# lukedan/libfluid

Measured on AMD Instinct MI355X. Metric: particle_steps_per_sec, higher is better.
Workload: dtype f32

## Files before the change

libfluid_amd/csrc/particles.hip:

```cpp
#include <math.h>

#include <algorithm>
#include <utility>

#include "common.h"
#include "pcg.h"

namespace {

__device__ inline bool solid_or_outside(const GridDims &g, const uint8_t *solid, int x, int y, int z) {
	if (!in_grid(g, x, y, z)) return true;
	return solid[blocked_index(g, x, y, z)] != 0;
}

__device__ inline void collide(const GridDims &g, const uint8_t *solid, double from[3], double to[3], double skin) {
	for (int bounce = 0; bounce < 3; ++bounce) {
		bool hit = false;
		double diff[3], inv[3], t[3];
		int cur[3], last[3], adv[3];
#pragma unroll
		for (int d = 0; d < 3; ++d) {
			cur[d] = (int)floor(from[d]);
			last[d] = (int)floor(to[d]);
			diff[d] = to[d] - from[d];
// ... 177 lines not shown
k_advect_collide(size_t n, ParticleSoA p, GridDims g, const uint8_t *solid, MoveParams mp, const uint8_t *coerce_map,
                 const float *src_vel, const uint8_t *tile_clear) {
	const size_t i = (size_t)blockIdx.x * blockDim.x + threadIdx.x;
	if (i < n) advect_one<COERCE>(i, p, g, solid, mp, coerce_map, src_vel, tile_clear);
}

#define AC_CHUNKS 8
template <bool COERCE>
__global__ void __launch_bounds__(256)
k_advect_collide_count(size_t n, ParticleSoA p, GridDims g, const uint8_t *solid, MoveParams mp, const uint8_t *coerce_map,
                       const float *src_vel, const uint8_t *tile_clear, uint32_t *tile_count, uint32_t *rank) {
	const int lane = threadIdx.x & 63;
	const size_t wave = ((size_t)blockIdx.x * blockDim.x + threadIdx.x) >> 6;
	const size_t i0 = wave * (64 * AC_CHUNKS) + lane;
	uint32_t tile[AC_CHUNKS], my_rank[AC_CHUNKS];
#pragma unroll
	for (int c = 0; c < AC_CHUNKS; ++c) {
		const size_t i = i0 + 64 * c;
		const uint32_t k = i < n ? advect_one<COERCE>(i, p, g, solid, mp, coerce_map, src_vel, tile_clear) : 0xFFFFFFFFu;
		tile[c] = k != 0xFFFFFFFFu ? k >> 9 : 0xFFFFFFFFu;
	}
	lfa_wave_tile_ranks(tile, tile_count, my_rank);
#pragma unroll
	for (int c = 0; c < AC_CHUNKS; ++c) {
		const size_t i = i0 + 64 * c;
		if (tile[c] != 0xFFFFFFFFu) rank[i] = my_rank[c];
	}
}

__device__ inline float hash_unit(uint32_t a, uint32_t b, uint32_t k) {
	uint32_t x = a * 0x9E3779B1u ^ (b + 0x7F4A7C15u) * 0x85EBCA77u ^ k * 0xC2B2AE3Du;
	x ^= x >> 15; x *= 0x2C1B3C6Du; x ^= x >> 12; x *= 0x297A2D39u; x ^= x >> 15;
	return (float)(x >> 8) * (2.0f / 16777216.0f) - 1.0f;
}

#define FT 11
#define FTX (2 * FT)
#define FT3 (FTX * FT * FT)
#define FT_STRIDE (FT3 + 1)
#define FT_INV 1.375f
#define FTX_INV 2.75f
#define FT_PL ((FT + CORR_PARTS - 1) / CORR_PARTS)
#define FB 13
#define FBX (FTX + 4)
#define FBZ (FT_PL + 2)
#define FB_N (FBX * FB * FBZ)
#define FB_ROWS (FB * FBZ)
#define FINE_CAP 5632
#define FINE_CAP_BIG 12288
#define FIDX_THREADS 512
#define FIDX_CNT (((FT3 + 1 + FIDX_THREADS - 1) / FIDX_THREADS) * FIDX_THREADS)
#define FIDX_STAGE 4608

__device__ inline int fine_coord(int l, float t) {
	const int f = (int)(((float)l + t) * FT_INV);
	return f < FT - 1 ? f : FT - 1;
}
__device__ inline int fine_coord_x(int l, float t) {
	const int f = (int)(((float)l + t) * FTX_INV);
	return f < FTX - 1 ? f : FTX - 1;
}
__device__ inline float4 fine_record(int lx, int ly, int lz, float t0, float t1, float t2, uint32_t index) {
	const uint32_t b0 = (__float_as_uint(t0) & 0x3FFFFFFFu) | ((uint32_t)(lx & 3) << 30);
	const uint32_t b1 = (__float_as_uint(t1) & 0x3FFFFFFFu) | ((uint32_t)(lx >> 2) << 31) | ((uint32_t)(ly & 1) << 30);
	const uint32_t b2 = (__float_as_uint(t2) & 0x3FFFFFFFu) | ((uint32_t)(lz & 1) << 31);
	return make_float4(__uint_as_float(b0), __uint_as_float(b1), __uint_as_float(b2), __uint_as_float(index));
}
__device__ inline void fine_decode_at(const float4 &r, int y0, int z0, float t[3], int l[3]) {
	const uint32_t b0 = __float_as_uint(r.x), b1 = __float_as_uint(r.y), b2 = __float_as_uint(r.z);
	t[0] = __uint_as_float(b0 & 0x3FFFFFFFu); t[1] = __uint_as_float(b1 & 0x3FFFFFFFu); t[2] = __uint_as_float(b2 & 0x3FFFFFFFu);
	l[0] = (int)(b0 >> 30) | ((int)(b1 >> 31) << 2);
	l[1] = y0 + ((y0 ^ (int)(b1 >> 30)) & 1);
	l[2] = z0 + ((z0 ^ (int)(b2 >> 31)) & 1);
}
__device__ inline void fine_decode(const float4 &r, int fy, int fz, float t[3], int l[3]) {
	fine_decode_at(r, (8 * fy) / FT, (8 * fz) / FT, t, l);
}

__global__ void __launch_bounds__(FIDX_THREADS)
k_build_fine_index(const int *ptiles, int n_ptiles, const uint32_t *key, const float *t0, const float *t1, const float *t2,
                   const uint32_t *tile_start, const uint32_t *tile_count, uint32_t *fine_start, float4 *spos, uint32_t *key_copy) {
	__shared__ uint32_t cnt[FIDX_CNT / 2];
	__shared__ uint32_t wsum[FIDX_THREADS / 64];
	__shared__ float4 stage[FIDX_STAGE];
	static_assert(FIDX_CNT % (2 * FIDX_THREADS) == 0 && FIDX_STAGE % FIDX_THREADS == 0 && FIDX_STAGE < 65536 && FIDX_CNT <= 4 * FIDX_STAGE,
	              "index kernel sizing");
	constexpr int PER = FIDX_CNT / FIDX_THREADS;
	uint32_t *cnt_big = (uint32_t *)stage;
	auto fine_of = [&](uint32_t i, int l[3], float t[3]) -> int {
		const uint32_t k = key[i];
		l[0] = (int)(k & 7); l[1] = (int)((k >> 3) & 7); l[2] = (int)((k >> 6) & 7);
		t[0] = t0[i]; t[1] = t1[i]; t[2] = t2[i];
		return fine_coord_x(l[0], t[0]) + FTX * (fine_coord(l[1], t[1]) + FT * fine_coord(l[2], t[2]));
	};
	constexpr int RPT = FIDX_STAGE / FIDX_THREADS;
	for (int slot = blockIdx.x; slot < n_ptiles; slot += gridDim.x) {
		const int tile = ptiles[slot];
		const uint32_t b = tile_start[tile], e = b + tile_count[tile];
		const bool staged = e - b <= FIDX_STAGE;
		if (staged) {
#pragma unroll
			for (int k = 0; k < PER / 2; ++k) cnt[threadIdx.x + FIDX_THREADS * k] = 0;
		} else {
#pragma unroll
			for (int k = 0; k < PER; ++k) cnt_big[threadIdx.x + FIDX_THREADS * k] = 0;
		}
		__syncthreads();
		uint32_t rf[RPT];
		float r0[RPT], r1[RPT], r2[RPT];
		if (staged) {
#pragma unroll
			for (int r = 0; r < RPT; ++r) {
				const uint32_t i = b + threadIdx.x + FIDX_THREADS * r;
				rf[r] = 0xFFFFFFFFu;
				if (i < e) {
					int l[3];
					float t[3];
					const int f = fine_of(i, l, t);
					rf[r] = ((uint32_t)f << 9) | (uint32_t)(l[0] | (l[1] << 3) | (l[2] << 6));
					r0[r] = t[0]; r1[r] = t[1]; r2[r] = t[2];
					atomicAdd(&cnt[f >> 1], 1u << (16 * (f & 1)));
				}
			}
		} else {
			for (uint32_t i = b + threadIdx.x; i < e; i += FIDX_THREADS) {
				int l[3];
				float t[3];
				atomicAdd(&cnt_big[fine_of(i, l, t)], 1u);
			}
		}
		__syncthreads();
		uint32_t c[PER], incl = 0;
#pragma unroll
		for (int k = 0; k < PER; ++k) {
			c[k] = staged ? (cnt[(PER / 2) * threadIdx.x + k / 2] >> (16 * (k & 1))) & 0xFFFFu : cnt_big[PER * threadIdx.x + k];
			incl += c[k];
		}
		const uint32_t sum = incl;
		const int lane = threadIdx.x & 63, wid = threadIdx.x >> 6;
#pragma unroll
		for (int o = 1; o < 64; o <<= 1) {
			uint32_t t = __shfl_up(incl, o, 64);
			if (lane >= o) incl += t;
		}
		if (lane == 63) wsum[wid] = incl;
		__syncthreads();
		uint32_t ex = incl - sum;
		for (int w = 0; w < wid; ++w) ex += wsum[w];
		__syncthreads();
#pragma unroll
		for (int k = 0; k < PER; ++k) {
			const int f = PER * threadIdx.x + k;
			if (!staged) cnt_big[f] = ex;
			else if (k & 1) cnt[f >> 1] = (ex - c[k - (k & 1)]) | (ex << 16);
			if (!staged && f <= FT3) fine_start[(size_t)tile * FT_STRIDE + f] = b + ex;
			ex += c[k];
		}
		__syncthreads();
		if (staged) {
#pragma unroll
			for (int r = 0; r < RPT; ++r)
				if (rf[r] != 0xFFFFFFFFu) {
					const uint32_t f = rf[r] >> 9;
					const uint32_t at = (atomicAdd(&cnt[f >> 1], 1u << (16 * (f & 1))) >> (16 * (f & 1))) & 0xFFFFu;
					stage[at] = fine_record((int)(rf[r] & 7), (int)((rf[r] >> 3) & 7), (int)((rf[r] >> 6) & 7), r0[r], r1[r], r2[r],
					                        b + threadIdx.x + FIDX_THREADS * r);
				}
			if (key_copy) {
#pragma unroll
				for (int r = 0; r < RPT; ++r)
					if (rf[r] != 0xFFFFFFFFu) key_copy[b + threadIdx.x + FIDX_THREADS * r] = ((uint32_t)tile << 9) | (rf[r] & 511u);
			}
			__syncthreads();
			for (int f = threadIdx.x; f <= FT3; f += FIDX_THREADS)
				fine_start[(size_t)tile * FT_STRIDE + f] = b + (f ? (cnt[(f - 1) >> 1] >> (16 * ((f - 1) & 1))) & 0xFFFFu : 0u);
			for (uint32_t k = threadIdx.x; k < e - b; k += FIDX_THREADS) spos[b + k] = stage[k];
		} else {
			for (uint32_t i = b + threadIdx.x; i < e; i += FIDX_THREADS) {
				int l[3];
				float t[3];
				const uint32_t at = atomicAdd(&cnt_big[fine_of(i, l, t)], 1u);
				spos[b + at] = fine_record(l[0], l[1], l[2], t[0], t[1], t[2], i);
				if (key_copy) key_copy[i] = key[i];
			}
		}
		__syncthreads();
	}
}

__device__ inline int fine_source(const GridDims &g, const uint32_t *tile_count, int tx, int ty, int tz, int gx, int gy, int gz, int &fx,
                                  int &fy, int &fz) {
	const int dx = gx < 0 ? -1 : (gx >= FTX ? 1 : 0), dy = gy < 0 ? -1 : (gy >= FT ? 1 : 0), dz = gz < 0 ? -1 : (gz >= FT ? 1 : 0);
	fx = gx - FTX * dx; fy = gy - FT * dy; fz = gz - FT * dz;
	const int x = tx + dx, y = ty + dy, z = tz + dz;
	if ((unsigned)x >= (unsigned)g.ntx || (unsigned)y >= (unsigned)g.nty || (unsigned)z >= (unsigned)g.ntz) return -1;
	const int tile = x + g.ntx * (y + g.nty * z);
	return tile_count[tile] ? tile : -1;
}

__device__ inline void correct_collide_record(size_t rk, const ParticleSoA &p, uint32_t *out_key, float *out_tx, float *out_ty, float *out_tz,
                                              const GridDims &g, const uint8_t *solid, const uint32_t *tile_count, const uint32_t *fine_start,
                                              const float4 *spos, const MoveParams &mp, const uint32_t *only_flagged, const int *tile_pslot,
                                              int p_off, const uint32_t *key_before) {
	const float4 me = spos[rk];
	const size_t i = __float_as_uint(me.w);
	const uint32_t key_i = key_before ? key_before[i] : p.key[i];
	if (key_i == 0xFFFFFFFFu) return;
	const int tile = (int)(key_i >> 9);
	const int l[3] = {(int)(key_i & 7), (int)((key_i >> 3) & 7), (int)((key_i >> 6) & 7)};
	const float t[3] = {__uint_as_float(__float_as_uint(me.x) & 0x3FFFFFFFu), __uint_as_float(__float_as_uint(me.y) & 0x3FFFFFFFu),
	                    __uint_as_float(__float_as_uint(me.z) & 0x3FFFFFFFu)};
	const int f[3] = {fine_coord_x(l[0], t[0]), fine_coord(l[1], t[1]), fine_coord(l[2], t[2])};
	if (only_flagged) {
		const int work = CORR_PARTS * (tile_pslot[tile] - p_off) + f[2] / FT_PL;
		if (!((only_flagged[1 + (work >> 5)] >> (work & 31)) & 1u)) return;
	}
	int tx, ty, tz;
	tile_coords(g, tile, tx, ty, tz);
	const int nn[3] = {g.nx, g.ny, g.nz};
	const float inv_re2 = (float)mp.inv_re2;
	double spring[3] = {0.0, 0.0, 0.0};
	for (int dz = -1; dz <= 1; ++dz)
		for (int dy = -1; dy <= 1; ++dy)
			for (int dx = -2; dx <= 2; ++dx) {
				int sf[3];
				const int src = fine_source(g, tile_count, tx, ty, tz, f[0] + dx, f[1] + dy, f[2] + dz, sf[0], sf[1], sf[2]);
				if (src < 0) continue;
				const uint32_t *fs = fine_start + (size_t)src * FT_STRIDE + (sf[0] + FTX * (sf[1] + FT * sf[2]));
				const uint32_t kb = fs[0], ke = fs[1];
				int stx, sty, stz;
				tile_coords(g, src, stx, sty, stz);
				for (uint32_t k = kb; k < ke; ++k) {
					const float4 rec = spos[k];
					if (__float_as_uint(rec.w) == (uint32_t)i) continue;
					float nt[3];
					int nl[3];
					fine_decode(rec, sf[1], sf[2], nt, nl);
					const float ddx = ((float)(8 * (tx - stx) + l[0] - nl[0]) + t[0]) - nt[0];
					const float ddy = ((float)(8 * (ty - sty) + l[1] - nl[1]) + t[1]) - nt[1];
					const float ddz = ((float)(8 * (tz - stz) + l[2] - nl[2]) + t[2]) - nt[2];
					const float d2 = ddx * ddx + ddy * ddy + ddz * ddz;
					if (d2 < 1e-12f) {
						const uint32_t j = __float_as_uint(rec.w);
						spring[0] += hash_unit((uint32_t)i, j, 0); spring[1] += hash_unit((uint32_t)i, j, 1);
						spring[2] += hash_unit((uint32_t)i, j, 2);
					} else {
						const float kl = 1.0f - d2 * inv_re2;
						if (kl > 0.0f) {
							const float fr = kl * kl * kl * rsqrtf(d2);
							spring[0] += (double)(fr * ddx); spring[1] += (double)(fr * ddy); spring[2] += (double)(fr * ddz);
						}
					}
				}
			}
	const int c[3] = {8 * tx + l[0], 8 * ty + l[1], 8 * tz + l[2]};
	double from[3], to[3];
#pragma unroll
	for (int d = 0; d < 3; ++d) {
		from[d] = (double)c[d] + (double)t[d];
		double x = from[d] + spring[d] * mp.corr;
		to[d] = x < 0.0 ? 0.0 : ((double)nn[d] < x ? (double)nn[d] : x);
	}
	if (mp.collide) collide(g, solid, from, to, mp.skin);
	int nc[3];
	float ntt[3];
#pragma unroll
	for (int d = 0; d < 3; ++d) split_position(to[d], nn[d], nc[d], ntt[d]);
	out_key[i] = blocked_index(g, nc[0], nc[1], nc[2]);
	out_tx[i] = ntt[0]; out_ty[i] = ntt[1]; out_tz[i] = ntt[2];
}

__global__ void __launch_bounds__(256)
k_correct_collide(size_t n, ParticleSoA p, uint32_t *out_key, float *out_tx, float *out_ty, float *out_tz, GridDims g,
                   const uint8_t *solid, const uint32_t *tile_count, const uint32_t *fine_start, const float4 *spos, MoveParams mp,
                   const uint32_t *only_flagged, const int *tile_pslot, int p_off, const uint32_t *key_before) {
	if (only_flagged && only_flagged[0] == 0) return;
	for (size_t rk = (size_t)blockIdx.x * blockDim.x + threadIdx.x; rk < n; rk += (size_t)gridDim.x * blockDim.x)
		correct_collide_record(rk, p, out_key, out_tx, out_ty, out_tz, g, solid, tile_count, fine_start, spos, mp, only_flagged, tile_pslot,
		                       p_off, key_before);
}

#ifdef CORR_PROFILE
__device__ unsigned long long g_corr_prof[8];
#define CORR_STAMP(k)                                                                   \
	do {                                                                                \
		if (!ONLY && threadIdx.x == 0) {                                                \
			const unsigned long long now_ = wall_clock64();                             \
			atomicAdd(&g_corr_prof[k], now_ - stamp_);                                  \
			stamp_ = now_;                                                              \
		}                                                                               \
	} while (0)
#else
#define CORR_STAMP(k) do { } while (0)
#endif
template <int CAP, bool ONLY>
__global__ void __launch_bounds__(ONLY ? CORR_THREADS_BIG : CORR_THREADS, 4)
k_correct_fine(const int *ptiles, int n_ptiles, uint32_t *out_key, float *out_tx, float *out_ty, float *out_tz, GridDims g,
                const uint8_t *solid, const uint32_t *tile_count, const uint32_t *fine_start, const float4 *spos, MoveParams mp,
                uint32_t *overflow_tiles, const uint8_t *tile_clear, const uint32_t *only) {
	constexpr int T = ONLY ? CORR_THREADS_BIG : CORR_THREADS;
	constexpr int CNT0 = ((FB_N + 1 + 2 * T - 1) / (2 * T)) * (2 * T);
	constexpr int CNT = ONLY && CNT0 < 4096 ? 4096 : CNT0;
	__shared__ float px[CAP], py[CAP], pz[CAP];
	__shared__ uint32_t fcnt2[CNT / 2];
	uint16_t *fcnt = (uint16_t *)fcnt2;
	__shared__ uint16_t foff[FB_N + 1];
	__shared__ __attribute__((aligned(16))) uint32_t rowd[FB_ROWS * 4];
	__shared__ uint32_t rowe[FB_ROWS];
	constexpr int ROW_NOT_OWN = -32768;
	__shared__ uint32_t ownoff[FT * FT_PL + 1];
	__shared__ int srct[27];
	__shared__ uint32_t wsum[T / 64];
	uint16_t *own = fcnt;
	static_assert(CNT > FB_N && CNT % (2 * T) == 0 && FBX % 2 == 0 && CAP < 32768 && CNT < 32768, "fcnt sizing");
	constexpr int PER = CNT / T;
	const int nn[3] = {g.nx, g.ny, g.nz};
	const int lane = threadIdx.x & 63, wid = threadIdx.x >> 6;
	if (ONLY && only[0] == 0) return;
	constexpr int SLICES = ONLY ? CORR_BIG_SLICES : 1;
	for (int item = blockIdx.x; item < SLICES * CORR_PARTS * n_ptiles; item += gridDim.x) {
		const int work = item / SLICES, slice = item % SLICES;
		if (ONLY && !((only[1 + (work >> 5)] >> (work & 31)) & 1u)) continue;
		const int tile = ptiles[work / CORR_PARTS], part = work % CORR_PARTS;
		int tx, ty, tz;
		tile_coords(g, tile, tx, ty, tz);
		const int own_lo = part * FT_PL, own_n = (own_lo + FT_PL <= FT ? FT_PL : FT - own_lo);
		const int gz0 = own_lo - 1;
		const int nzb = own_n + 2;
		const int nrows = FB * nzb, nown_rows = FT * (nzb - 2);
		const bool open_water = (tile_clear[tile] & 1) != 0;
		const bool lean = open_water && mp.collide && tx >= 1 && ty >= 1 && tz >= 1 && 8 * tx + 16 <= g.nx && 8 * ty + 16 <= g.ny &&
		                  8 * tz + 16 <= g.nz;
		__syncthreads();
#ifdef CORR_PROFILE
		unsigned long long stamp_ = wall_clock64();
		if (!ONLY && threadIdx.x == 0) atomicAdd(&g_corr_prof[7], 1ull);
#endif
		uint32_t tid = threadIdx.x;
		asm volatile("" : "+v"(tid));
		if (tid < 27) {
			int fx, fy, fz;
			srct[tid] = fine_source(g, tile_count, tx, ty, tz, FTX * ((int)tid % 3 - 1), FT * (((int)tid / 3) % 3 - 1), FT * ((int)tid / 9 - 1), fx,
			                        fy, fz);
		}
		__syncthreads();
		constexpr int ROUNDS = CNT / (2 * T), KEPT = ROUNDS - 1 < 2 ? ROUNDS - 1 : 2;
#pragma unroll
		for (int k = 0; k < ROUNDS; ++k) {
			const int p = (int)(k >= KEPT ? tid : threadIdx.x) + T * k;
			uint32_t cnt0 = 0, cnt1 = 0, src0 = 0;
			if (p < (FBX / 2) * nrows) {
				const int bx = 2 * (p % (FBX / 2)), row = p / (FBX / 2), by = row % FB, bz = row / FB;
				const int gx = bx - 2, gy = by - 1, gz = gz0 + bz;
				const int dx = gx < 0 ? 0 : (gx >= FTX ? 2 : 1), dy = gy < 0 ? 0 : (gy >= FT ? 2 : 1), dz = gz < 0 ? 0 : (gz >= FT ? 2 : 1);
				const int src = srct[dx + 3 * dy + 9 * dz];
				if (src >= 0) {
					const uint32_t fid = (uint32_t)((gx - FTX * (dx - 1)) + FTX * ((gy - FT * (dy - 1)) + FT * (gz - FT * (dz - 1))));
					const uint32_t *fs = fine_start + ((uint32_t)src * FT_STRIDE + fid);
					src0 = fs[0];
					const uint32_t mid = fs[1];
					cnt0 = mid - src0;
					cnt1 = fs[2] - mid;
				}
				if (bx == 0 || bx == 2 || bx == FBX - 2) rowd[row * 4 + (bx == 0 ? 0 : (bx == 2 ? 1 : 2))] = src0;
			}
			fcnt2[p] = (cnt0 < 0xFFFFu ? cnt0 : 0xFFFFu) | ((cnt1 < 0xFFFFu ? cnt1 : 0xFFFFu) << 16);
		}
		__syncthreads();
		uint32_t c4[PER], sum = 0;
#pragma unroll
		for (int k = 0; k < PER; ++k) {
			c4[k] = fcnt[PER * threadIdx.x + k];
			sum += c4[k];
		}
		uint32_t incl = sum;
#pragma unroll
		for (int o = 1; o < 64; o <<= 1) {
			uint32_t t = __shfl_up(incl, o, 64);
			if (lane >= o) incl += t;
		}
		if (lane == 63) wsum[wid] = incl;
		__syncthreads();
		uint32_t woff = 0, total = 0;
		for (int w = 0; w < T / 64; ++w) {
			if (w < wid) woff += wsum[w];
			total += wsum[w];
		}
		if (total > (uint32_t)CAP) {
			if (threadIdx.x == 0 && slice == 0) {
				atomicOr(&overflow_tiles[1 + (work >> 5)], 1u << (work & 31));
				atomicAdd(&overflow_tiles[0], 1u);
			}
			continue;
		}
		{
			uint32_t ex = woff + incl - sum;
#pragma unroll
			for (int k = 0; k < PER; ++k) {
				const int f = PER * threadIdx.x + k;
				if (f <= FB_N) foff[f] = (uint16_t)ex;
				ex += c4[k];
			}
		}
		__syncthreads();
		uint32_t own_total = 0, own_first = 0;
		{
			uint32_t len = 0;
			if (tid < (unsigned)nown_rows) {
				const int row = (1 + (int)tid % FT) + FB * (1 + (int)tid / FT);
				len = (uint32_t)foff[row * FBX + FBX - 2] - (uint32_t)foff[row * FBX + 2];
			}
			uint32_t in2 = len;
#pragma unroll
			for (int o = 1; o < 64; o <<= 1) {
				uint32_t t = __shfl_up(in2, o, 64);
				if (lane >= o) in2 += t;
			}
			if (lane == 63) wsum[wid] = in2;
			__syncthreads();
			uint32_t wo = 0;
			for (int w = 0; w < T / 64; ++w) {
				if (w < wid) wo += wsum[w];
				own_total += wsum[w];
			}
			own_first = wo + in2 - len;
			if (tid < (unsigned)nown_rows) ownoff[tid] = own_first;
			if (tid == 0) ownoff[nown_rows] = own_total;
		}
		const bool listed = own_total <= (uint32_t)CNT;
		if (tid < (unsigned)nrows) {
			const int r = (int)tid, by = r % FB, bz = r / FB;
			const int gy = by - 1, gz = gz0 + bz;
			const int dy = gy < 0 ? -1 : (gy >= FT ? 1 : 0), dz = gz < 0 ? -1 : (gz >= FT ? 1 : 0);
			const int fy = gy - FT * dy, fz = gz - FT * dz;
			const uint32_t d0 = foff[r * FBX], d1 = foff[r * FBX + 2], d2 = foff[r * FBX + FBX - 2];
			uint32_t *rd = rowd + r * 4;
			rd[0] -= d0; rd[1] -= d1; rd[2] -= d2;
			rd[3] = d1 | (d2 << 16);
			rowe[r] = (uint32_t)((8 * fy) / FT) | ((uint32_t)((8 * fz) / FT) << 3) | ((uint32_t)(8 * (dy + 1)) << 6) |
			          ((uint32_t)(8 * (dz + 1)) << 11) | ((uint32_t)ROW_NOT_OWN << 16);
		}
		__syncthreads();
		if (listed && tid < (unsigned)nown_rows) {
			const int row = (1 + (int)tid % FT) + FB * (1 + (int)tid / FT);
			rowe[row] = (rowe[row] & 0xFFFFu) | ((own_first - (uint32_t)foff[row * FBX + 2]) << 16);
		}
		__syncthreads();
		CORR_STAMP(0);
		{
			static_assert(FB_ROWS <= 128, "two row starts per lane");
			const int rl = (int)(tid & 63u);
			const uint32_t rs_lo = rl < nrows ? (uint32_t)foff[rl * FBX] : 0xFFFFFFFFu;
			const uint32_t rs_hi = rl + 64 < nrows ? (uint32_t)foff[(rl + 64) * FBX] : 0xFFFFFFFFu;
			auto row_of = [&](uint32_t s) -> int {
				return (int)__popcll(__ballot(rs_lo <= s)) + (int)__popcll(__ballot(rs_hi <= s)) - 1;
			};
			auto locate = [&](uint32_t slot, int r_first, int r_last, uint32_t &src, int &rs) {
				int r = r_first;
				const int span = r_last - r_first;
				for (int step = span ? 1 << (31 - __builtin_clz(span)) : 0; step; step >>= 1) {
					const int c = r + step;
					if (c <= r_last && (uint32_t)foff[c * FBX] <= slot) r = c;
				}
				const uint4 d = *(const uint4 *)(rowd + r * 4);
				const int seg = slot < (d.w & 0xFFFFu) ? 0 : (slot < (d.w >> 16) ? 1 : 2);
				src = (seg == 0 ? d.x : (seg == 1 ? d.y : d.z)) + slot;
				rs = r | (seg << 8);
			};
			auto put = [&](uint32_t slot, const float4 &rec, int rs) {
				const int r = rs & 255, seg = rs >> 8;
				const uint32_t d = rowe[r];
				const int ob = (int)d >> 16;
				float t[3];
				int l[3];
				fine_decode_at(rec, (int)(d & 7u), (int)((d >> 3) & 7u), t, l);
				px[slot] = (float)(8 * (seg - 1) + l[0]) + t[0];
				py[slot] = (float)((int)((d >> 6) & 31u) - 8 + l[1]) + t[1];
				pz[slot] = (float)((int)((d >> 11) & 31u) - 8 + l[2]) + t[2];
				if (seg == 1 && ob != ROW_NOT_OWN) own[ob + (int)slot] = (uint16_t)slot;
			};
			const uint32_t wave0 = (uint32_t)__builtin_amdgcn_readfirstlane((int)(threadIdx.x & ~63u));
			for (uint32_t w0 = wave0; w0 < total; w0 += CORR_STAGE_DEPTH * T) {
				uint32_t src[CORR_STAGE_DEPTH];
				int rs[CORR_STAGE_DEPTH];
				float4 rec[CORR_STAGE_DEPTH];
#pragma unroll
				for (int u = 0; u < CORR_STAGE_DEPTH; ++u) {
					const uint32_t wu = w0 + u * T, slot = wu + lane;
					src[u] = 0; rs[u] = 0;
					if (wu < total) {
						const uint32_t last = wu + 63 < total ? wu + 63 : total - 1;
						const int r_first = row_of(wu), r_last = row_of(last);
						if (slot < total) locate(slot, r_first, r_last, src[u], rs[u]);
					}
				}
#pragma unroll
				for (int u = 0; u < CORR_STAGE_DEPTH; ++u) rec[u] = spos[src[u]];
#pragma unroll
				for (int u = 0; u < CORR_STAGE_DEPTH; ++u) {
					const uint32_t slot = w0 + u * T + lane;
					if (slot < total) put(slot, rec[u], rs[u]);
				}
			}
		}
		__syncthreads();
		CORR_STAMP(1);
#ifdef CORR_PROFILE
		if (!ONLY && threadIdx.x == 0) { atomicAdd(&g_corr_prof[5], (unsigned long long)total); atomicAdd(&g_corr_prof[6], (unsigned long long)own_total); }
#endif
		for (uint32_t w = threadIdx.x + T * slice; w < own_total; w += T * SLICES) {
			uint32_t me;
			if (listed) {
				me = own[w];
			} else {
				int lo = 0, hi = nown_rows - 1;
				while (lo < hi) {
					const int mid = (lo + hi + 1) >> 1;
					if (ownoff[mid] <= w) lo = mid;
					else hi = mid - 1;
				}
				me = (uint32_t)foff[((1 + lo % FT) + FB * (1 + lo / FT)) * FBX + 2] + (w - ownoff[lo]);
			}
#ifdef CORR_PROFILE
			const unsigned long long w0_ = wall_clock64();
#endif
			const float mx = px[me], my = py[me], mz = pz[me];
			int fx = (int)(mx * FTX_INV), fy = (int)(my * FT_INV), fz = (int)(mz * FT_INV);
			fx = fx < FTX - 1 ? fx : FTX - 1; fy = fy < FT - 1 ? fy : FT - 1; fz = fz < FT - 1 ? fz : FT - 1;
			const int bx = fx + 2, by = fy + 1, bz = fz - gz0;
			float sx = 0.f, sy = 0.f, sz = 0.f;
			typedef float f2 __attribute__((ext_vector_type(2)));
			f2 s2x = 0.f, s2y = 0.f, s2z = 0.f;
			const float inv_re2 = (float)mp.inv_re2;
			uint32_t j = 0xFFFFFFFFu;
			const uint32_t myrow = by + FB * bz;
			const uint32_t grec = rowd[myrow * 4 + 1] + me;
			auto pair2 = [&](uint32_t q, f2 qx, f2 qy, f2 qz) {
				const f2 dx = mx - qx, dy = my - qy, dz = mz - qz;
				const f2 d2 = __builtin_elementwise_fma(dz, dz, __builtin_elementwise_fma(dy, dy, dx * dx));
				const f2 kl = __builtin_elementwise_fma(-d2, (f2)inv_re2, (f2)1.0f);
				if (kl.x > 0.0f || kl.y > 0.0f) {
#pragma unroll
					for (int k = 0; k < 2; ++k) {
						const float d2k = k ? d2.y : d2.x, klk = k ? kl.y : kl.x;
						if (!(klk > 0.0f)) continue;
						if (d2k < 1e-12f) {
							if (q + k != me) {
								if (j == 0xFFFFFFFFu) j = __float_as_uint(spos[grec].w);
								sx += hash_unit(j, q + k, 0); sy += hash_unit(j, q + k, 1); sz += hash_unit(j, q + k, 2);
							}
						} else {
							const float f = klk * klk * klk * rsqrtf(d2k);
							sx += f * (k ? dx.y : dx.x); sy += f * (k ? dy.y : dy.x); sz += f * (k ? dz.y : dz.x);
						}
					}
				}
			};
			auto walk = [&](auto &&p2, auto &&p2_centre) {
				for (int dz = -1; dz <= 1; ++dz)
					for (int dy = -1; dy <= 1; ++dy) {
						const int rowf = FBX * ((by + dy) + FB * (bz + dz)) + bx;
						const uint32_t b = foff[rowf - 2], e = foff[rowf + 3];
						auto run = [&](auto &&pp) {
							uint32_t q = b;
							for (; q + 4 <= e; q += 4) {
								const float x0 = px[q], x1 = px[q + 1], x2 = px[q + 2], x3 = px[q + 3];
								const float y0 = py[q], y1 = py[q + 1], y2 = py[q + 2], y3 = py[q + 3];
								const float z0 = pz[q], z1 = pz[q + 1], z2 = pz[q + 2], z3 = pz[q + 3];
								pp(q, f2{x0, x1}, f2{y0, y1}, f2{z0, z1});
								pp(q + 2, f2{x2, x3}, f2{y2, y3}, f2{z2, z3});
							}
							if (q + 2 <= e) {
								pp(q, f2{px[q], px[q + 1]}, f2{py[q], py[q + 1]}, f2{pz[q], pz[q + 1]});
								q += 2;
							}
							if (q < e) pp(q, f2{px[q], 1e6f}, f2{py[q], 1e6f}, f2{pz[q], 1e6f});
						};
						if (dy == 0 && dz == 0) run(p2_centre);
						else run(p2);
					}
			};
			float d2_min = 1.0f;
			uint32_t n_tiny = 0;
			auto fast = [&](f2 qx, f2 qy, f2 qz) -> f2 {
				const f2 dx = mx - qx, dy = my - qy, dz = mz - qz;
				const f2 d2 = __builtin_elementwise_fma(dz, dz, __builtin_elementwise_fma(dy, dy, __builtin_elementwise_fma(dx, dx, (f2)1e-30f)));
				f2 kl;
				kl.x = __builtin_amdgcn_fmed3f(__builtin_fmaf(-d2.x, inv_re2, 1.0f), 0.0f, 1.0f);
				kl.y = __builtin_amdgcn_fmed3f(__builtin_fmaf(-d2.y, inv_re2, 1.0f), 0.0f, 1.0f);
				f2 f = kl * kl * kl;
				f.x *= __builtin_amdgcn_rsqf(d2.x);
				f.y *= __builtin_amdgcn_rsqf(d2.y);
				s2x = __builtin_elementwise_fma(f, dx, s2x);
				s2y = __builtin_elementwise_fma(f, dy, s2y);
				s2z = __builtin_elementwise_fma(f, dz, s2z);
				return d2;
			};
			walk([&](uint32_t, f2 qx, f2 qy, f2 qz) {
					     const f2 d2 = fast(qx, qy, qz);
					     d2_min = fminf(d2_min, fminf(d2.x, d2.y));
				     },
				     [&](uint32_t, f2 qx, f2 qy, f2 qz) {
					     const f2 d2 = fast(qx, qy, qz);
					     n_tiny += (d2.x < 1e-12f ? 1u : 0u) + (d2.y < 1e-12f ? 1u : 0u);
				     });
			if (d2_min < 1e-12f || n_tiny != 1u) {
				s2x = 0.f; s2y = 0.f; s2z = 0.f;
				walk(pair2, pair2);
			}
			sx += s2x.x + s2x.y;
			sy += s2y.x + s2y.y;
			sz += s2z.x + s2z.y;
#ifdef CORR_PROFILE
			if (!ONLY && threadIdx.x == 0) atomicAdd(&g_corr_prof[4], wall_clock64() - w0_);
#endif
			float tme[3];
			int lme[3];
			const float4 rec = spos[grec];
			const uint32_t yz = rowe[myrow];
			fine_decode_at(rec, (int)(yz & 7u), (int)((yz >> 3) & 7u), tme, lme);
			const uint32_t jj = __float_as_uint(rec.w);
			const int c[3] = {8 * tx + lme[0], 8 * ty + lme[1], 8 * tz + lme[2]};
			const double spring[3] = {(double)sx, (double)sy, (double)sz};
			double from[3], to[3];
#pragma unroll
			for (int d = 0; d < 3; ++d) {
				from[d] = (double)c[d] + (double)tme[d];
				to[d] = from[d] + spring[d] * mp.corr;
			}
			if (!(lean && fabs(to[0] - from[0]) < 7.0 && fabs(to[1] - from[1]) < 7.0 && fabs(to[2] - from[2]) < 7.0)) {
#pragma unroll
				for (int d = 0; d < 3; ++d) to[d] = to[d] < 0.0 ? 0.0 : ((double)nn[d] < to[d] ? (double)nn[d] : to[d]);
				if (mp.collide) {
					if (!open_water || fabs(to[0] - from[0]) >= 7.0 || fabs(to[1] - from[1]) >= 7.0 || fabs(to[2] - from[2]) >= 7.0)
						collide(g, solid, from, to, mp.skin);
					else
						collide_walls_only(g, to, mp.skin);
				}
			}
			int nc[3];
			float nt[3];
#pragma unroll
			for (int d = 0; d < 3; ++d) split_position(to[d], nn[d], nc[d], nt[d]);
			out_key[jj] = blocked_index(g, nc[0], nc[1], nc[2]);
			out_tx[jj] = nt[0]; out_ty[jj] = nt[1]; out_tz[jj] = nt[2];
		}
#ifdef CORR_PROFILE
		CORR_STAMP(2);
		__syncthreads();
		CORR_STAMP(3);
#endif
	}
}

}
#ifdef CORR_PROFILE
extern "C" int lfa_debug_corr_prof(uint64_t out[8], int reset) {
	unsigned long long h[8] = {0};
	if (hipMemcpyFromSymbol(h, HIP_SYMBOL(g_corr_prof), sizeof h) != hipSuccess) return -1;
	for (int i = 0; i < 8; ++i) out[i] = h[i];
	if (reset) {
		unsigned long long z[8] = {0};
		if (hipMemcpyToSymbol(HIP_SYMBOL(g_corr_prof), z, sizeof z) != hipSuccess) return -1;
	}
	return 0;
}
#endif

static MoveParams move_params(const lfa_sim *s, double dt) {
	MoveParams mp;
	const double h = s->prm.cell_size, re = h / sqrt(2.0);
	mp.dt_over_h = dt / h;
	mp.skin = s->prm.boundary_skin_width / h;
	mp.corr = dt * s->prm.correction_stiffness * re / h;
	mp.inv_re2 = h * h / (re * re);
	mp.collide = 1;
	mp.c_home = s->c_home_valid ? s->c_home : nullptr;
	mp.c_home_stride = s->c_home_cap;
	return mp;
}


namespace {
__global__ void k_mark_coerce(const uint32_t *cell, const uint32_t *src1, size_t n, uint8_t *map) {
	const size_t i = (size_t)blockIdx.x * blockDim.x + threadIdx.x;
	if (i < n) map[cell[i]] = (uint8_t)src1[i];
}
__global__ void k_source_need(const uint32_t *cell, const uint32_t *lo, const uint32_t *target, size_t n, const uint32_t *cell_count,
                              const uint32_t *tile_flag, uint32_t *need) {
	const size_t i = (size_t)blockIdx.x * blockDim.x + threadIdx.x;
	if (i >= n) return;
	const uint32_t b = cell[i];
	const uint32_t have = lo[i] != 0xFFFFFFFFu ? lo[i] : (tile_flag[b >> 9] ? cell_count[b] : 0u);
	need[i] = target[i] > have ? target[i] - have : 0u;
}
__global__ void k_source_need_scatter(const uint32_t *need, const uint32_t *gidx, size_t n, float *all) {
	const size_t i = (size_t)blockIdx.x * blockDim.x + threadIdx.x;
	if (i < n) all[gidx[i]] = (float)need[i];
}
__global__ void k_source_need_gather(const float *all, size_t n, uint32_t *need) {
	const size_t i = (size_t)blockIdx.x * blockDim.x + threadIdx.x;
	if (i < n) need[i] = (uint32_t)all[i];
}
__device__ inline uint64_t mix64(uint64_t x) {
	x ^= x >> 30; x *= 0xBF58476D1CE4E5B9ull;
	x ^= x >> 27; x *= 0x94D049BB133111EBull;
	x ^= x >> 31;
	return x;
}
__global__ void k_source_seed(const uint32_t *cell, const uint32_t *src_of, const uint32_t *need, const uint32_t *off, size_t n,
                              const float *src_vel, ParticleSoA p, size_t base, uint64_t seed, uint64_t id_base) {
	const size_t i = (size_t)blockIdx.x * blockDim.x + threadIdx.x;
	if (i >= n) return;
	const uint32_t cnt = need[i], b = cell[i];
	const float *vel = src_vel + 3 * src_of[i];
	for (uint32_t j = 0; j < cnt; ++j) {
		const size_t d = base + off[i] + j;
		p.key[d] = b;
#pragma unroll
		for (int a = 0; a < 3; ++a) {
			const uint64_t r = mix64(seed + ((id_base + (uint64_t)(d - base)) * 3ull + (uint64_t)a + 1ull) * 0x9E3779B97F4A7C15ull + ((uint64_t)b << 40));
			float t = (float)(r >> 40) * (1.0f / 16777216.0f);
			p.t[a][d] = t;
			p.v[a][d] = vel[a];
		}
		particle_zero_c_set_id(p, d, (uint32_t)(id_base + (uint64_t)(d - base)));
	}
}
}

extern "C" int lfa_clear_sources(lfa_sim *s) {
	if (!s) return LFA_E_INVALID;
	s->sources.clear();
	s->sources_valid = false;
	return LFA_OK;
}

extern "C" int lfa_add_source(lfa_sim *s, const int32_t *xyz, uint64_t k, const double velocity[3], uint64_t root, int active,
                              int coerce_velocity) {
	if (!s || (!xyz && k) || !velocity) return LFA_E_INVALID;
	if (s->sources.size() >= 254) return lfa_fail(s, LFA_E_UNSUPPORTED, "more than 254 fluid sources");
	if (root > 16) return lfa_fail(s, LFA_E_INVALID, "target_density_cubic_root %llu: more than 4096 particles per cell", (unsigned long long)root);
	for (uint64_t i = 0; i < k; ++i)
		if (!in_grid(s->g, xyz[3 * i], xyz[3 * i + 1], xyz[3 * i + 2]))
			return lfa_fail(s, LFA_E_INVALID, "source cell (%d, %d, %d) outside the grid", xyz[3 * i], xyz[3 * i + 1], xyz[3 * i + 2]);
	lfa_sim::SourceHost h;
	h.xyz.assign(xyz, xyz + 3 * k);
	for (int d = 0; d < 3; ++d) h.vel[d] = velocity[d];
// ... 729 lines not shown
```

Baseline: 5.166 billion.

## Derive fine-cell offsets from per-row runs instead of a full block scan

Replaces the per-cell count array and the full-block prefix scan with a per-row scan over three contiguous source runs. Because particles in fine_start are already sorted, each cell's offset can be taken directly as its start minus a per-row base, which removes one scan, several barriers and the separate own-row scan. It also reorders the work-item mapping so groups of eight tiles interleave their parts. The offset derivation relies on runs being contiguous per source tile, and register pressure rises from the per-round fs0/fs1 arrays.

After: 5.294 billion (median of 6 runs). 1.02x the previous value.

```diff
diff --git a/libfluid_amd/csrc/particles.hip b/libfluid_amd/csrc/particles.hip
--- a/libfluid_amd/csrc/particles.hip
+++ b/libfluid_amd/csrc/particles.hip
@@ -503,24 +503,25 @@
 	constexpr int CNT0 = ((FB_N + 1 + 2 * T - 1) / (2 * T)) * (2 * T);
 	constexpr int CNT = ONLY && CNT0 < 4096 ? 4096 : CNT0;
 	__shared__ float px[CAP], py[CAP], pz[CAP];
-	__shared__ uint32_t fcnt2[CNT / 2];
-	uint16_t *fcnt = (uint16_t *)fcnt2;
-	__shared__ uint16_t foff[FB_N + 1];
+	__shared__ uint16_t own[CNT];
+	__shared__ uint32_t foff2[(FB_N + 2) / 2];
+	const uint16_t *foff = (const uint16_t *)foff2;
 	__shared__ __attribute__((aligned(16))) uint32_t rowd[FB_ROWS * 4];
 	__shared__ uint32_t rowe[FB_ROWS];
 	constexpr int ROW_NOT_OWN = -32768;
 	__shared__ uint32_t ownoff[FT * FT_PL + 1];
 	__shared__ int srct[27];
 	__shared__ uint32_t wsum[T / 64];
-	uint16_t *own = fcnt;
-	static_assert(CNT > FB_N && CNT % (2 * T) == 0 && FBX % 2 == 0 && CAP < 32768 && CNT < 32768, "fcnt sizing");
-	constexpr int PER = CNT / T;
+	static_assert(CNT > FB_N && CNT % (2 * T) == 0 && FBX % 2 == 0 && CAP < 32768 && CNT < 32768, "own list and cell rounds sizing");
 	const int nn[3] = {g.nx, g.ny, g.nz};
 	const int lane = threadIdx.x & 63, wid = threadIdx.x >> 6;
 	if (ONLY && only[0] == 0) return;
 	constexpr int SLICES = ONLY ? CORR_BIG_SLICES : 1;
 	for (int item = blockIdx.x; item < SLICES * CORR_PARTS * n_ptiles; item += gridDim.x) {
-		const int work = item / SLICES, slice = item % SLICES;
+		int work = item / SLICES;
+		const int slice = item % SLICES;
+		if (!ONLY && (item / (8 * CORR_PARTS)) * 8 + 8 <= n_ptiles)
+			work = CORR_PARTS * ((item / (8 * CORR_PARTS)) * 8 + item % 8) + (item % (8 * CORR_PARTS)) / 8;
 		if (ONLY && !((only[1 + (work >> 5)] >> (work & 31)) & 1u)) continue;
 		const int tile = ptiles[work / CORR_PARTS], part = work % CORR_PARTS;
 		int tx, ty, tz;
@@ -546,47 +547,62 @@
 		}
 		__syncthreads();
 		constexpr int ROUNDS = CNT / (2 * T), KEPT = ROUNDS - 1 < 2 ? ROUNDS - 1 : 2;
+		uint32_t fs0[ROUNDS], fs1[ROUNDS];
+		int fbase[ROUNDS];
 #pragma unroll
 		for (int k = 0; k < ROUNDS; ++k) {
 			const int p = (int)(k >= KEPT ? tid : threadIdx.x) + T * k;
-			uint32_t cnt0 = 0, cnt1 = 0, src0 = 0;
+			fs0[k] = 0; fs1[k] = 0; fbase[k] = -1;
 			if (p < (FBX / 2) * nrows) {
 				const int bx = 2 * (p % (FBX / 2)), row = p / (FBX / 2), by = row % FB, bz = row / FB;
 				const int gx = bx - 2, gy = by - 1, gz = gz0 + bz;
 				const int dx = gx < 0 ? 0 : (gx >= FTX ? 2 : 1), dy = gy < 0 ? 0 : (gy >= FT ? 2 : 1), dz = gz < 0 ? 0 : (gz >= FT ? 2 : 1);
 				const int src = srct[dx + 3 * dy + 9 * dz];
+				fbase[k] = row * 4 + dx;
 				if (src >= 0) {
 					const uint32_t fid = (uint32_t)((gx - FTX * (dx - 1)) + FTX * ((gy - FT * (dy - 1)) + FT * (gz - FT * (dz - 1))));
 					const uint32_t *fs = fine_start + ((uint32_t)src * FT_STRIDE + fid);
-					src0 = fs[0];
-					const uint32_t mid = fs[1];
-					cnt0 = mid - src0;
-					cnt1 = fs[2] - mid;
+					fs0[k] = fs[0]; fs1[k] = fs[1];
 				}
-				if (bx == 0 || bx == 2 || bx == FBX - 2) rowd[row * 4 + (bx == 0 ? 0 : (bx == 2 ? 1 : 2))] = src0;
-			}
-			fcnt2[p] = (cnt0 < 0xFFFFu ? cnt0 : 0xFFFFu) | ((cnt1 < 0xFFFFu ? cnt1 : 0xFFFFu) << 16);
+			}
+		}
+		static_assert(FB_ROWS <= 128 && T >= 256, "the rows are the first two waves; wsum holds two sums of each scan");
+		uint32_t run_at[3] = {0, 0, 0}, run_n[3] = {0, 0, 0}, row_incl = 0, own_incl = 0, row_n = 0, own_len = 0;
+		int own_row = -1;
+		uint32_t rowe_lo = 0;
+		if (tid < 128u) {
+			const int r = (int)tid, by = r % FB, bz = r / FB;
+			const int gy = by - 1, gz = gz0 + bz;
+			const int dy = gy < 0 ? -1 : (gy >= FT ? 1 : 0), dz = gz < 0 ? -1 : (gz >= FT ? 1 : 0);
+			const int fy = gy - FT * dy, fz = gz - FT * dz;
+			if (r < nrows) {
+				const uint32_t frow = (uint32_t)(FTX * (fy + FT * fz));
+#pragma unroll
+				for (int seg = 0; seg < 3; ++seg) {
+					const int src = srct[seg + 3 * (dy + 1) + 9 * (dz + 1)];
+					if (src >= 0) {
+						const uint32_t *fs = fine_start + ((uint32_t)src * FT_STRIDE + frow + (seg == 0 ? FTX - 2 : 0));
+						run_at[seg] = fs[0];
+						run_n[seg] = fs[seg == 1 ? FTX : 2] - run_at[seg];
+					}
+				}
+				row_n = run_n[0] + run_n[1] + run_n[2];
+				if (by >= 1 && by <= FT && bz >= 1 && bz <= nzb - 2) {
+					own_row = (by - 1) + FT * (bz - 1);
+					own_len = run_n[1];
+				}
+				rowe_lo = (uint32_t)((8 * fy) / FT) | ((uint32_t)((8 * fz) / FT) << 3) | ((uint32_t)(8 * (dy + 1)) << 6) | ((uint32_t)(8 * (dz + 1)) << 11);
+			}
+			row_incl = row_n; own_incl = own_len;
+#pragma unroll
+			for (int o = 1; o < 64; o <<= 1) {
+				const uint32_t t = __shfl_up(row_incl, o, 64), u = __shfl_up(own_incl, o, 64);
+				if (lane >= o) { row_incl += t; own_incl += u; }
+			}
+			if (lane == 63) { wsum[wid] = row_incl; wsum[2 + wid] = own_incl; }
 		}
 		__syncthreads();
-		uint32_t c4[PER], sum = 0;
-#pragma unroll
-		for (int k = 0; k < PER; ++k) {
-			c4[k] = fcnt[PER * threadIdx.x + k];
-			sum += c4[k];
-		}
-		uint32_t incl = sum;
-#pragma unroll
-		for (int o = 1; o < 64; o <<= 1) {
-			uint32_t t = __shfl_up(incl, o, 64);
-			if (lane >= o) incl += t;
-		}
-		if (lane == 63) wsum[wid] = incl;
-		__syncthreads();
-		uint32_t woff = 0, total = 0;
-		for (int w = 0; w < T / 64; ++w) {
-			if (w < wid) woff += wsum[w];
-			total += wsum[w];
-		}
+		const uint32_t total = wsum[0] + wsum[1], own_total = wsum[2] + wsum[3];
 		if (total > (uint32_t)CAP) {
 			if (threadIdx.x == 0 && slice == 0) {
 				atomicOr(&overflow_tiles[1 + (work >> 5)], 1u << (work & 31));
@@ -594,57 +610,27 @@
 			}
 			continue;
 		}
-		{
-			uint32_t ex = woff + incl - sum;
-#pragma unroll
-			for (int k = 0; k < PER; ++k) {
-				const int f = PER * threadIdx.x + k;
-				if (f <= FB_N) foff[f] = (uint16_t)ex;
-				ex += c4[k];
-			}
-		}
-		__syncthreads();
-		uint32_t own_total = 0, own_first = 0;
-		{
-			uint32_t len = 0;
-			if (tid < (unsigned)nown_rows) {
-				const int row = (1 + (int)tid % FT) + FB * (1 + (int)tid / FT);
-				len = (uint32_t)foff[row * FBX + FBX - 2] - (uint32_t)foff[row * FBX + 2];
-			}
-			uint32_t in2 = len;
-#pragma unroll
-			for (int o = 1; o < 64; o <<= 1) {
-				uint32_t t = __shfl_up(in2, o, 64);
-				if (lane >= o) in2 += t;
-			}
-			if (lane == 63) wsum[wid] = in2;
-			__syncthreads();
-			uint32_t wo = 0;
-			for (int w = 0; w < T / 64; ++w) {
-				if (w < wid) wo += wsum[w];
-				own_total += wsum[w];
-			}
-			own_first = wo + in2 - len;
-			if (tid < (unsigned)nown_rows) ownoff[tid] = own_first;
-			if (tid == 0) ownoff[nown_rows] = own_total;
-		}
 		const bool listed = own_total <= (uint32_t)CNT;
 		if (tid < (unsigned)nrows) {
-			const int r = (int)tid, by = r % FB, bz = r / FB;
-			const int gy = by - 1, gz = gz0 + bz;
-			const int dy = gy < 0 ? -1 : (gy >= FT ? 1 : 0), dz = gz < 0 ? -1 : (gz >= FT ? 1 : 0);
-			const int fy = gy - FT * dy, fz = gz - FT * dz;
-			const uint32_t d0 = foff[r * FBX], d1 = foff[r * FBX + 2], d2 = foff[r * FBX + FBX - 2];
-			uint32_t *rd = rowd + r * 4;
-			rd[0] -= d0; rd[1] -= d1; rd[2] -= d2;
-			rd[3] = d1 | (d2 << 16);
-			rowe[r] = (uint32_t)((8 * fy) / FT) | ((uint32_t)((8 * fz) / FT) << 3) | ((uint32_t)(8 * (dy + 1)) << 6) |
-			          ((uint32_t)(8 * (dz + 1)) << 11) | ((uint32_t)ROW_NOT_OWN << 16);
-		}
+			const uint32_t d0 = (wid ? wsum[0] : 0u) + row_incl - row_n, d1 = d0 + run_n[0], d2 = d1 + run_n[1];
+			*(uint4 *)(rowd + tid * 4) = make_uint4(run_at[0] - d0, run_at[1] - d1, run_at[2] - d2, d1 | (d2 << 16));
+			uint32_t ob = (uint32_t)ROW_NOT_OWN;
+			if (own_row >= 0) {
+				const uint32_t own_first = (wid ? wsum[2] : 0u) + own_incl - own_len;
+				ownoff[own_row] = own_first;
+				if (listed) ob = own_first - d1;
+			}
+			rowe[tid] = rowe_lo | (ob << 16);
+		}
+		if (tid == 0) ownoff[nown_rows] = own_total;
 		__syncthreads();
-		if (listed && tid < (unsigned)nown_rows) {
-			const int row = (1 + (int)tid % FT) + FB * (1 + (int)tid / FT);
-			rowe[row] = (rowe[row] & 0xFFFFu) | ((own_first - (uint32_t)foff[row * FBX + 2]) << 16);
+#pragma unroll
+		for (int k = 0; k < ROUNDS; ++k) {
+			const int p = (int)(k >= KEPT ? tid : threadIdx.x) + T * k;
+			if (p < (FB_N + 2) / 2) {
+				const uint32_t base = fbase[k] >= 0 ? rowd[fbase[k]] : 0u - total;
+				foff2[p] = ((fs0[k] - base) & 0xFFFFu) | ((fs1[k] - base) << 16);
+			}
 		}
 		__syncthreads();
 		CORR_STAMP(0);
```
